# khiner/MeshEditor

Hardware: AMD Instinct MI355X
Metric: eigenpairs/sec (K/M assembly + 50-mode solve, 100k-tet mesh) (higher is better)
Workload: dtype f64; 1 GPU; cube_s100k: Kuhn mesh 105456 tets / 446631 DOF, NumModes=50 NumFemModes=65, P=10 excitation points, one mesh per GPU; eigenpairs_per_mesh=65, kept_modes_per_mesh=50, parallelism=mesh-per-gpu x1

## Files before the change

### mesheditor_amd/csrc/lab/mh_lab.hip

```cpp
#include "../mh_common.h"
#include "modalhip_lab.h"

#include <algorithm>

void mh_elementwise_apply(mh_context *ctx, const mh_system *sys, double sigma, const double *x, double *y, uint32_t w);

namespace {
constexpr int TB = 256;
__global__ void k_lab_ref_to_panel(const double *__restrict__ x, const uint32_t *__restrict__ perm, uint32_t nnodes, uint32_t width, double *__restrict__ panel) {
    const size_t i = size_t(blockIdx.x) * blockDim.x + threadIdx.x;
    if (i >= size_t(nnodes) * 3 * width) return;
    const uint32_t c = uint32_t(i % width), comp = uint32_t((i / width) % 3), node = uint32_t(i / (size_t(3) * width));
    panel[i] = x[size_t(c) * (size_t(3) * nnodes) + size_t(3) * perm[node] + comp];
}
__global__ void k_lab_panel_to_ref(const double *__restrict__ panel, const uint32_t *__restrict__ perm, uint32_t nnodes, uint32_t width, double *__restrict__ y) {
    const size_t i = size_t(blockIdx.x) * blockDim.x + threadIdx.x;
    if (i >= size_t(nnodes) * 3 * width) return;
    const uint32_t c = uint32_t(i % width), comp = uint32_t((i / width) % 3), node = uint32_t(i / (size_t(3) * width));
    y[size_t(c) * (size_t(3) * nnodes) + size_t(3) * perm[node] + comp] = panel[i];
}
}

namespace {
typedef float f4_stream __attribute__((ext_vector_type(4)));
// ... 223 lines not shown
    size_t bad = differing(one.x, hx);
    for (size_t r = 0; r < n; ++r)
        for (uint32_t c = 0; c < nc; ++c) {
            double ref = 0, mag = 0;
            for (uint32_t k = 0; k < m; ++k) {
                const double s = k < wa ? hx[r * b + map[k]] : k < wa + wb ? hw[r * wb + (k - wa)] : hp[r * wb + (k - wa - wb)];
                ref += s * hc[size_t(k) * nc + c];
                mag += std::abs(s * hc[size_t(k) * nc + c]);
            }
            const double got = c < wa ? one.xn[r * pitch + c] : one.p[r * wb + (c - wa)];
            bad += !(std::abs(got - ref) <= 2.0 * m * 2.3e-16 * mag);
        }
    std::vector<double> want = hx;
    size_t written = 0;
    for (size_t r = 0; r < n; ++r)
        for (uint32_t k = 0; k < wa; ++k) {
            want[r * b + map[k]] = one.xn[r * pitch + k];
            written += want[r * b + map[k]] != hx[r * b + map[k]];
        }
    if (written < n * wa / 2) mh_throw(MH_EHIP, "mapped update check: the update left %zu of %zu entries as they were", n * wa - written, n * size_t(wa));
    bad += differing(two.xn, one.xn) + differing(two.x, want) + differing(two.p, one.p);
    return double(bad);
}
}

extern "C" {
int mhl_context_bench_dense(mh_context *ctx, int kind, uint64_t n, uint32_t wa, uint32_t wb, uint32_t reps, double *avg_ms) {
    if (!ctx || !avg_ms || n == 0 || wa == 0 || wb == 0 || reps == 0 || kind < 0 || kind > 3) return MH_EINVAL;
    try {
        HIP_CHECK(hipSetDevice(ctx->device));
        std::lock_guard<std::mutex> lock(mh_solve_mutex());
        if (kind >= 2) {
            *avg_ms = lab_mapped_update_mismatches(ctx, kind == 3, n, wa, wb);
            return MH_OK;
        }
        DevArray<double> x(ctx, n * wa), y(ctx, n * wb), g(ctx, size_t(wa + wb) * (wa + wb)), z(ctx, n * wa);
        std::vector<double> h(n * std::max(wa, wb));
        for (size_t i = 0; i < h.size(); ++i) h[i] = double((i * 2654435761u) % 1000) * 1e-3 - 0.5;
        x.upload(h.data(), n * wa);
        y.upload(h.data(), n * wb);
        g.upload(h.data(), g.count);
        HIP_CHECK(hipStreamSynchronize(ctx->stream));
        auto run = [&]() {
            if (kind == 0) mh_gram(ctx, n, x, wa, y, wb, g, wa);
            else mh_combine(ctx, n, x, wa, y, wb, nullptr, 0, g, wa, z, wa, nullptr);
        };
        run();
        hipEvent_t e0, e1;
        HIP_CHECK(hipEventCreate(&e0));
        HIP_CHECK(hipEventCreate(&e1));
        HIP_CHECK(hipEventRecord(e0, ctx->stream));
        for (uint32_t r = 0; r < reps; ++r) run();
        HIP_CHECK(hipEventRecord(e1, ctx->stream));
// ... 513 lines not shown
```

### mesheditor_amd/csrc/mh_common.h

```cpp
#pragma once
#include "../../include/modalhip.h"

#include <hip/hip_runtime.h>
#include <rocblas/rocblas.h>
#include <rocsolver/rocsolver.h>

#include <algorithm>
#include <cstdarg>
#include <cstdio>
#include <cstdlib>
#include <cstring>
#include <iterator>
#include <limits>
#include <atomic>
#include <map>
#include <memory>
#include <mutex>
#include <stdexcept>
#include <string>
#include <vector>

struct MhError : std::runtime_error {
    int code;
    MhError(int c, const std::string &m) : std::runtime_error(m), code(c) {}
};

[[noreturn]] inline void mh_throw(int code, const char *fmt, ...) {
    char buf[512];
    va_list ap;
    va_start(ap, fmt);
    vsnprintf(buf, sizeof(buf), fmt, ap);
    va_end(ap);
    throw MhError(code, buf);
}

#define HIP_CHECK(expr)                                                                                         \
    do {                                                                                                        \
        hipError_t e_ = (expr);                                                                                 \
        if (e_ != hipSuccess) mh_throw(MH_EHIP, "%s failed: %s (%s:%d)", #expr, hipGetErrorString(e_), __FILE__, __LINE__); \
    } while (0)
#define ROCBLAS_CHECK(expr)                                                                                     \
    do {                                                                                                        \
// ... 175 lines not shown
        bytes_idle += it->second;
        live.erase(it);
        while (bytes_idle > cap && !free_blocks.empty()) {
            auto oldest = free_blocks.begin();
            for (auto f = free_blocks.begin(); f != free_blocks.end(); ++f)
                if (f->second.stamp < oldest->second.stamp) oldest = f;
            (void)hipFree(oldest->second.p);
            bytes_idle -= oldest->first;
            bytes_reserved -= oldest->first;
            free_blocks.erase(oldest);
        }
    }
    void trim() {
        for (auto &kv : free_blocks) (void)hipFree(kv.second.p), bytes_reserved -= kv.first;
        free_blocks.clear();
        bytes_idle = 0;
    }
    ~DevicePool() {
        trim();
        for (auto &kv : live) (void)hipFree(kv.first);
    }
};

struct mh_context {
    int device{0};
    int cu_count{256};
    hipStream_t stream{nullptr};
    hipStream_t aux_stream{nullptr};
    bool aux_stream_ready() {
        if (!aux_stream && hipStreamCreateWithFlags(&aux_stream, hipStreamNonBlocking) != hipSuccess) aux_stream = nullptr;
        if (aux_stream && !blas_aux) {
            if (rocblas_create_handle(&blas_aux) != rocblas_status_success) blas_aux = nullptr;
            else if (rocblas_set_stream(blas_aux, aux_stream) != rocblas_status_success) {
                (void)rocblas_destroy_handle(blas_aux);
                blas_aux = nullptr;
            }
        }
        return aux_stream != nullptr && blas_aux != nullptr;
    }
    hipStream_t aux2_stream{nullptr};
    std::vector<hipEvent_t> ahead_ev;
    bool aux2_stream_ready(size_t events = 0) {
        if (!aux2_stream && hipStreamCreateWithFlags(&aux2_stream, hipStreamNonBlocking) != hipSuccess) aux2_stream = nullptr, (void)hipGetLastError();
        while (aux2_stream && ahead_ev.size() < events) {
            hipEvent_t e = nullptr;
            if (hipEventCreateWithFlags(&e, hipEventDisableTiming) != hipSuccess) { (void)hipGetLastError(); return false; }
            ahead_ev.push_back(e);
        }
        return aux2_stream != nullptr;
    }
    rocblas_handle blas{nullptr};
    rocblas_handle blas_aux{nullptr};
    DevicePool pool;
    std::string last_error;
    hipEvent_t ev0{nullptr}, ev1{nullptr};
    void *gram_ws{nullptr};
    size_t gram_ws_bytes{0};
    uint32_t *iota{nullptr};
    unsigned long long *sytrd_xch{nullptr};
    uint32_t sytrd_epoch{0};
    int *sytrd_flag{nullptr};
    unsigned long long *sytrd_xch_wide{nullptr};
    uint32_t sytrd_epoch_wide{0};
    bool exchange_disabled{false};
    uint32_t sytrd_redos{0};
    unsigned long long *rr_check{nullptr};
    struct MhRrTrace *rr_trace{nullptr};
    bool time_kernels{false};
    std::vector<std::pair<hipEvent_t, hipEvent_t>> timer_events;
    std::vector<double> timer_work;
    std::vector<int> timer_class;
    size_t timer_used{0};
    struct ClassTotals {
        double ms{0}, work{0};
        uint64_t launches{0};
    } totals[MH_KERNEL_CLASSES];
// ... 5 lines not shown
    size_t slot{0};
    TimedLaunch(mh_context *c, int kernel_class, double work) : ctx(c), on(c->time_kernels) {
        if (!on) return;
        if (ctx->timer_used == ctx->timer_events.size()) {
            hipEvent_t a, b;
            HIP_CHECK(hipEventCreate(&a));
            HIP_CHECK(hipEventCreate(&b));
            ctx->timer_events.emplace_back(a, b);
            ctx->timer_work.push_back(0);
            ctx->timer_class.push_back(0);
        }
        slot = ctx->timer_used++;
        ctx->timer_work[slot] = work;
        ctx->timer_class[slot] = kernel_class;
        HIP_CHECK(hipEventRecord(ctx->timer_events[slot].first, ctx->stream));
    }
    ~TimedLaunch() {
        if (on) (void)hipEventRecord(ctx->timer_events[slot].second, ctx->stream);
    }
    TimedLaunch(const TimedLaunch &) = delete;
    TimedLaunch &operator=(const TimedLaunch &) = delete;
};

template<typename T> struct DevArray {
    mh_context *ctx{nullptr};
    T *ptr{nullptr};
    size_t count{0};
    bool owned{true};
    DevArray() = default;
    DevArray(mh_context *c, size_t n) { reset(c, n); }
    DevArray(const DevArray &) = delete;
    DevArray &operator=(const DevArray &) = delete;
    DevArray(DevArray &&o) noexcept : ctx(o.ctx), ptr(o.ptr), count(o.count), owned(o.owned) { o.ptr = nullptr; o.count = 0; o.owned = true; }
    DevArray &operator=(DevArray &&o) noexcept {
        if (this != &o) {
            free();
            ctx = o.ctx; ptr = o.ptr; count = o.count; owned = o.owned;
            o.ptr = nullptr; o.count = 0; o.owned = true;
        }
        return *this;
    }
    void alias_of(const DevArray &o) {
        free();
        ctx = o.ctx; ptr = o.ptr; count = o.count;
        owned = false;
    }
    ~DevArray() { free(); }
    void reset(mh_context *c, size_t n) {
        free();
        ctx = c;
        count = n;
        ptr = n ? static_cast<T *>(c->pool.alloc(n * sizeof(T))) : nullptr;
        static const bool poison = getenv("MH_TEST") && strstr(getenv("MH_TEST"), "poison");
        if (poison && ptr) (void)hipMemsetAsync(ptr, 0xff, n * sizeof(T), c->stream);
    }
    void free() {
        if (ptr && ctx && owned) ctx->pool.release(ptr);
        ptr = nullptr;
        count = 0;
        owned = true;
    }
    T *get() const { return ptr; }
    operator T *() const { return ptr; }
    void zero() const { if (ptr) HIP_CHECK(hipMemsetAsync(ptr, 0, count * sizeof(T), ctx->stream)); }
    void upload(const T *src, size_t n) const { HIP_CHECK(hipMemcpyAsync(ptr, src, n * sizeof(T), hipMemcpyHostToDevice, ctx->stream)); }
    void download(T *dst, size_t n) const {
        HIP_CHECK(hipMemcpyAsync(dst, ptr, n * sizeof(T), hipMemcpyDeviceToHost, ctx->stream));
        HIP_CHECK(hipStreamSynchronize(ctx->stream));
    }
    std::vector<T> to_host() const {
        std::vector<T> h(count);
        if (count) download(h.data(), count);
        return h;
    }
};

struct MhLevelStructure {
    uint32_t n_nodes{0};
    uint64_t n_blocks{0};
    DevArray<uint32_t> row_ptr, col;
    DevArray<uint32_t> seg, pay;
};
struct mh_structure {
    mh_context *ctx{nullptr};
    uint32_t n_points{0}, kept_tets{0}, n_nodes{0}, n_edges{0};
    DevArray<double> points;
    DevArray<uint32_t> tets;
    DevArray<uint32_t> elem_nodes_ref, elem_nodes, elem_p1;
    DevArray<double> elem_basis;
    DevArray<uint32_t> perm, inv_perm;
    bool relative{false};
    double origin[3]{0, 0, 0};
// ... 199 lines not shown
```

### mesheditor_amd/csrc/mh_dense.hip

```cpp
#include "mh_common.h"

#include <optional>

#include <map>

static bool mh_test_own_gemm() {
    static const bool on = getenv("MH_TEST") && strstr(getenv("MH_TEST"), "own_gemm");
    return on;
}
namespace {
constexpr int KC = 32;

typedef double double4_t __attribute__((ext_vector_type(4)));

__host__ __device__ inline int pad_pitch(int w) {
    int p = ((w + 15) / 16) * 16;
    if ((p % 32) != 16) p += 16;
    return p;
}

template<int TI, int TJ, int GI, int GJ, int KS, int OCC>
__global__ void __launch_bounds__(GI * GJ * KS * 64) __attribute__((amdgpu_waves_per_eu(OCC, OCC))) k_gram_blocked(const double *__restrict__ X, int ldx, int wa, const double *__restrict__ Y, int ldy, const uint32_t *__restrict__ ymap, int wb,
                                                                  size_t n, size_t rows_per_wg, double *__restrict__ partial) {
    extern __shared__ __attribute__((aligned(16))) double smem[];
// ... 1210 lines not shown
    if (multi && m >= 32) {
        constexpr int G = MH_SYTRD_GROUPS;
        constexpr size_t words = SYTRD_XCH_WORDS + SYTRD_ACK_WORDS;
        if (!ctx->sytrd_xch) {
            ctx->sytrd_xch = static_cast<unsigned long long *>(ctx->pool.alloc(words * sizeof(unsigned long long) + 64));
            HIP_CHECK(hipMemsetAsync(ctx->sytrd_xch, 0, words * sizeof(unsigned long long) + 64, ctx->stream));
        }
        if ((++ctx->sytrd_epoch & 0x7fffffu) == 0) {
            ctx->sytrd_epoch = 1;
            HIP_CHECK(hipMemsetAsync(ctx->sytrd_xch, 0, words * sizeof(unsigned long long) + 64, ctx->stream));
        }
        ctx->sytrd_flag = reinterpret_cast<int *>(ctx->sytrd_xch + words);
        HIP_CHECK(hipMemsetAsync(ctx->sytrd_flag, 0, sizeof(int), ctx->stream));
        k_sytrd_multi<G><<<8 * G, 256, 0, ctx->stream>>>(a, int(m), d, e, tau, ctx->sytrd_xch, ctx->sytrd_epoch, ctx->sytrd_flag);
    } else if (variant == 3) k_sytrd_regs<<<1, 512, 0, ctx->stream>>>(a, int(m), d, e, tau);
    else if (fused) k_sytrd_small_fused<<<1, MH_SYTRD_THREADS, 0, ctx->stream>>>(a, int(m), d, e, tau);
    else k_sytrd_small<<<1, 1024, 0, ctx->stream>>>(a, int(m), d, e, tau);
    KERNEL_CHECK();
}

bool mh_sytrd_gave_up(mh_context *ctx) {
    if (!ctx->sytrd_flag) return false;
    int flag = 0;
    HIP_CHECK(hipMemcpyAsync(&flag, ctx->sytrd_flag, sizeof(flag), hipMemcpyDeviceToHost, ctx->stream));
    HIP_CHECK(hipStreamSynchronize(ctx->stream));
    return flag != 0;
}

namespace {
template<int Q, int PF>
__global__ void __launch_bounds__(64) k_apply_q(const double *__restrict__ A, const double *__restrict__ tau, int m, double *__restrict__ Z, int ldz) {
    const int lane = threadIdx.x;
    double *zc = Z + size_t(blockIdx.x) * ldz;
    double z[Q], v[PF][Q], tk[PF];
#pragma unroll
    for (int q = 0; q < Q; ++q) z[q] = lane + 64 * q < m ? zc[lane + 64 * q] : 0.0;
    auto load = [&](int k, double (&dst)[Q], double &t) {
        t = k >= 0 ? tau[k] : 0.0;
#pragma unroll
        for (int q = 0; q < Q; ++q) {
            const int i = lane + 64 * q;
            dst[q] = (k >= 0 && i < m && i > k + 1) ? A[size_t(k) * m + i] : (i == k + 1 ? 1.0 : 0.0);
        }
    };
#pragma unroll
    for (int u = 0; u < PF; ++u) load(m - 2 - u, v[u], tk[u]);
    for (int k0 = m - 2; k0 >= 0; k0 -= PF) {
#pragma unroll
// ... 471 lines not shown
    if (m <= 256 || m > WIDE_T || k < 1 || k > 256 || k > m) return false;
    const size_t km = size_t(k) * m;
    double *xt = work, *xt2 = xt + km, *ufac = xt2 + km, *g = ufac + 3 * km, *linv = g + size_t(k) * k, *qual = linv + size_t(k) * k;
    k_tridiag_values<3><<<k, 256, 0, ctx->stream>>>(d, e, int(m), w);
    KERNEL_CHECK();
    k_tridiag_invit<<<div_up(k, 64), 64, 0, ctx->stream>>>(d, e, int(m), int(k), w, xt, ufac);
    KERNEL_CHECK();
    DevArray<int> info4_array(ctx, 4);
    int *info4 = info4_array.get();
    HIP_CHECK(hipMemsetAsync(info4, 0, 4 * sizeof(int), ctx->stream));
    for (int pass = 0; pass < 2; ++pass) {
        const double *src = pass == 0 ? xt : xt2;
        mh_small_gemm(ctx, false, true, k, k, m, 1.0, src, k, src, k, 0.0, g, k);
        mh_potrf(ctx, g, k, k, info4 + 2 * pass);
        HIP_CHECK(hipMemsetAsync(linv, 0, size_t(k) * k * sizeof(double), ctx->stream));
        ROCBLAS_CHECK(rocblas_dtrtri(ctx->blas, rocblas_fill_lower, rocblas_diagonal_non_unit, rocblas_int(k), g, rocblas_int(k), linv, rocblas_int(k)));
        if (pass == 0) mh_small_gemm(ctx, false, false, k, m, k, 1.0, linv, k, src, k, 0.0, xt2, k);
        else mh_small_gemm(ctx, true, true, m, k, k, 1.0, src, k, linv, k, 0.0, z, ldz);
    }
    HIP_CHECK(hipMemsetAsync(qual, 0, sizeof(double), ctx->stream));
    k_tridiag_residual<<<k, 256, 0, ctx->stream>>>(d, e, int(m), w, z, int(ldz), reinterpret_cast<unsigned long long *>(qual));
    KERNEL_CHECK();
    int hinfo[4] = {0, 0, 0, 0};
    HIP_CHECK(hipMemcpyAsync(quality_host, qual, sizeof(double), hipMemcpyDeviceToHost, ctx->stream));
    HIP_CHECK(hipMemcpyAsync(hinfo, info4, sizeof(hinfo), hipMemcpyDeviceToHost, ctx->stream));
    HIP_CHECK(hipStreamSynchronize(ctx->stream));
    if (hinfo[0] != 0 || hinfo[2] != 0) *quality_host = std::numeric_limits<double>::quiet_NaN();
    return true;
}

namespace {
__global__ void __launch_bounds__(256) k_potrf_small(double *__restrict__ A, int w, int *__restrict__ info) {
    extern __shared__ __attribute__((aligned(16))) double L[];
    __shared__ int s_fail;
    const int tid = threadIdx.x, pitch = w + 1;
    for (int idx = tid; idx < w * w; idx += 256) L[(idx / w) * pitch + idx % w] = A[idx];
    if (tid == 0) s_fail = 0;
    __syncthreads();
    for (int k = 0; k < w; ++k) {
        const double akk = L[k * pitch + k];
        if (!(akk > 0.0)) {
            if (tid == 0) s_fail = k + 1;
            break;
        }
        const double d = sqrt(akk), inv = 1.0 / d;
        __syncthreads();
        for (int i = k + tid; i < w; i += 256) L[k * pitch + i] = i == k ? d : L[k * pitch + i] * inv;
        __syncthreads();
        const int rem = w - k - 1;
// ... 382 lines not shown
```

### mesheditor_amd/csrc/mh_eigs.hip

```cpp
#include "mh_common.h"

#include <algorithm>
#include <cmath>
#include <memory>
#include <condition_variable>
#include <mutex>
#include <numeric>
#include <optional>
#include <type_traits>

__global__ void k_shift_values(const double *kval, const double *mval, size_t nblocks, double sigma, double *aval, float *aval32);
__global__ void k_diag_inverse(const uint32_t *row_ptr, const uint32_t *col, const double *aval, uint32_t nnodes, double *dinv);
__global__ void k_coarse_matrix(const uint32_t *row_ptr, const uint32_t *col, const double *aval, const double *tmat, const uint32_t *agg_of, const uint32_t *agg_ptr,
                                const uint32_t *agg_nodes, uint32_t nagg, double *a0);
__global__ void k_fix_coarse_diag(double *a0, uint32_t n0, double rel);

namespace {
constexpr int TB = 256;

std::mutex g_solve_mutex;
struct Switches {
    bool verbose = getenv("MH_VERBOSE") != nullptr;
    bool fp32_prec = !(getenv("MH_PRECOND_FP64") && atoi(getenv("MH_PRECOND_FP64")) != 0);
    int deg2 = 0, deg1 = 0, gamma = 0;
    double cheb_ratio = 0.0, cheb_ratio1 = 0.0;
    bool test_sytrd_giveup = getenv("MH_TEST") && strstr(getenv("MH_TEST"), "sytrd_giveup");
    bool no_tridiag_wide = getenv("MH_TEST") && strstr(getenv("MH_TEST"), "no_tridiag_wide");
    bool test_last_resort = getenv("MH_TEST") && strstr(getenv("MH_TEST"), "last_resort");
    bool test_coarse_pivot = getenv("MH_TEST") && strstr(getenv("MH_TEST"), "coarse_pivot");
    bool test_selfcheck_fail = getenv("MH_TEST") && strstr(getenv("MH_TEST"), "selfcheck_fail");
    bool lmax_low = getenv("MH_TEST") && strstr(getenv("MH_TEST"), "lmax_low");
    bool potrf_chain = getenv("MH_TEST") && strstr(getenv("MH_TEST"), "potrf_chain");
    bool no_poly_start = getenv("MH_TEST") && strstr(getenv("MH_TEST"), "no_poly_start");
    bool fresh_structure = getenv("MH_TEST") && strstr(getenv("MH_TEST"), "fresh_structure");
    bool copy_passes = getenv("MH_TEST") && strstr(getenv("MH_TEST"), "copy_passes");
    Switches() {
        if (const char *c = getenv("MH_CYCLE")) {
            double v[5] = {0, 0, 0, 0, 0};
            sscanf(c, "%lf,%lf,%lf,%lf,%lf", &v[0], &v[1], &v[2], &v[3], &v[4]);
            deg2 = std::max(0, int(v[0])), deg1 = std::max(0, int(v[1])), gamma = std::max(0, int(v[2]));
            cheb_ratio = v[3];
            cheb_ratio1 = v[4];
        }
    }
};
const Switches &switches() {
    static const Switches s;
    return s;
}
constexpr int kPowerIterations = 20;
constexpr uint32_t kPrecondColumns = 256;
constexpr uint32_t kSkipP = 4;
constexpr uint32_t kGuardPercent = 10;
constexpr float kFlatShape = 1e-4f;
constexpr size_t kDenseLastResort = 12288;
constexpr int kLastResortCg = 8;

struct PhaseLock {
// ... 572 lines not shown
bool sytrd_gave_up(mh_context *ctx, int flag, double *gA, const double *saved, uint32_t m) {
    if (!flag && !switches().test_sytrd_giveup) return false;
    ++ctx->sytrd_redos;
    HIP_CHECK(hipMemcpyAsync(gA, saved, size_t(m) * m * sizeof(double), hipMemcpyDeviceToDevice, ctx->stream));
    return true;
}
bool accept_partial(mh_context *ctx, double quality, double *evals, const double *lam, uint32_t nwant) {
    if (!(quality < 1e-10)) return false;
    HIP_CHECK(hipMemcpyAsync(evals, lam, size_t(nwant) * sizeof(double), hipMemcpyDeviceToDevice, ctx->stream));
    return true;
}

int eig_tridiag_small(mh_context *ctx, double *gA, uint32_t m, double *evals, double *ework, DevArray<int> &info, uint32_t nwant, std::vector<double> *host_evals) {
    DevArray<double> z(ctx, size_t(m) * m), tau(ctx, m);
    const bool partial = nwant && nwant < m;
    DevArray<double> zl(ctx, partial ? size_t(m) * nwant : 0);
    double *zres = z.get();
    uint32_t ncols = m;
    HIP_CHECK(hipMemcpyAsync(z.get(), gA, size_t(m) * m * sizeof(double), hipMemcpyDeviceToDevice, ctx->stream));
    for (int attempt = 0; attempt < 2; ++attempt) {
        mh_sytrd_small(ctx, gA, m, evals, ework, tau, attempt == 0 ? -1 : 0);
        int gave_up = 0;
        const bool flagged = attempt == 0 && ctx->sytrd_flag;
        if (flagged) HIP_CHECK(hipMemcpyAsync(&gave_up, ctx->sytrd_flag, sizeof(int), hipMemcpyDeviceToHost, ctx->stream));
        if (partial) {
            DevArray<double> wv(ctx, 2 * m + 8), ufac(ctx, size_t(3) * m * nwant);
            double *zout = attempt == 0 ? zl.get() : z.get();
            if (mh_tridiag_lowest(ctx, evals, ework, m, nwant, wv, zout, m, ufac, wv.get() + m, wv.get() + m + 8)) {
                double qv[5] = {1, 0, 0, 0, 0};
                std::vector<double> lam_host(host_evals ? nwant : 0);
                HIP_CHECK(hipMemcpyAsync(qv, wv.get() + m, sizeof(qv), hipMemcpyDeviceToHost, ctx->stream));
                if (host_evals) HIP_CHECK(hipMemcpyAsync(lam_host.data(), wv.get(), size_t(nwant) * sizeof(double), hipMemcpyDeviceToHost, ctx->stream));
                HIP_CHECK(hipStreamSynchronize(ctx->stream));
                if (flagged && sytrd_gave_up(ctx, gave_up, gA, z, m)) continue;
                if (switches().verbose)
                    fprintf(stderr, "[rr] tridiagonal m %u lowest %u: residual / ||T|| %.2e; us: multisection %.0f, inverse iteration %.0f, Gram-Schmidt %.0f, output %.0f\n", m,
                            nwant, qv[0], qv[1] * 0.01, qv[2] * 0.01, qv[3] * 0.01, qv[4] * 0.01);
                if (ctx->rr_trace) ctx->rr_trace->quality = qv[0];
                if (accept_partial(ctx, qv[0], evals, wv, nwant)) {
                    if (host_evals) host_evals->swap(lam_host);
                    zres = zout, ncols = nwant;
                    break;
                }
            }
        }
        if (flagged) {
            HIP_CHECK(hipStreamSynchronize(ctx->stream));
            if (sytrd_gave_up(ctx, gave_up, gA, z, m)) continue;
        }
        ROCBLAS_CHECK(rocsolver_dstedc(ctx->blas, rocblas_evect_tridiagonal, m, evals, ework, z, m, info));
        if (const int hinfo = host_info(info)) return hinfo;
        break;
    }
    if (ctx->rr_trace) ctx->rr_trace->solver = ncols < m ? MhRrTrace::SMALL_PARTIAL : MhRrTrace::SMALL_STEDC;
    mh_apply_q(ctx, gA, tau, m, zres, m, ncols);
    if (zres == zl.get()) rr_selfcheck(ctx, z.get(), m, zres, m, evals, ncols);
    HIP_CHECK(hipMemcpyAsync(gA, zres, size_t(m) * ncols * sizeof(double), hipMemcpyDeviceToDevice, ctx->stream));
    return 0;
}

std::optional<int> eig_tridiag_wide(mh_context *ctx, double *gA, uint32_t m, double *evals, double *ework, DevArray<int> &info, uint32_t nwant) {
    DevArray<double> z(ctx, size_t(m) * m), saved(ctx, size_t(m) * m), tau(ctx, m);
    HIP_CHECK(hipMemcpyAsync(saved.get(), gA, size_t(m) * m * sizeof(double), hipMemcpyDeviceToDevice, ctx->stream));
    mh_sytrd_wide(ctx, gA, m, evals, ework, tau);
    int gave_up = 0;
    HIP_CHECK(hipMemcpyAsync(&gave_up, ctx->sytrd_flag, sizeof(int), hipMemcpyDeviceToHost, ctx->stream));
    HIP_CHECK(hipStreamSynchronize(ctx->stream));
    if (sytrd_gave_up(ctx, gave_up, gA, saved, m)) return std::nullopt;
    if (nwant && nwant < m && nwant <= 256 && !switches().no_tridiag_wide) {
        DevArray<double> work(ctx, size_t(5) * nwant * m + size_t(2) * nwant * nwant + 8), lam(ctx, nwant);
        double quality = 1.0;
        if (mh_tridiag_lowest_wide(ctx, evals, ework, m, nwant, lam, z, m, work, info, &quality)) {
            if (switches().verbose) fprintf(stderr, "[rr] tridiagonal m %u lowest %u (wide): residual / ||T|| %.2e\n", m, nwant, quality);
            if (ctx->rr_trace) ctx->rr_trace->quality = quality;
            if (accept_partial(ctx, quality, evals, lam, nwant)) {
                if (ctx->rr_trace) ctx->rr_trace->solver = MhRrTrace::WIDE_PARTIAL;
                mh_apply_q(ctx, gA, tau, m, z, m, nwant);
                rr_selfcheck(ctx, saved.get(), m, z, m, evals, nwant);
                HIP_CHECK(hipMemcpyAsync(gA, z.get(), size_t(m) * nwant * sizeof(double), hipMemcpyDeviceToDevice, ctx->stream));
                HIP_CHECK(hipStreamSynchronize(ctx->stream));
                return 0;
            }
        }
    }
    ROCBLAS_CHECK(rocsolver_dstedc(ctx->blas, rocblas_evect_tridiagonal, m, evals, ework, z, m, info));
    if (const int hinfo = host_info(info)) return hinfo;
    ROCBLAS_CHECK(rocsolver_dormtr(ctx->blas, rocblas_side_left, rocblas_fill_lower, rocblas_operation_none, m, m, gA, m, tau, z, m));
    if (ctx->rr_trace) ctx->rr_trace->solver = MhRrTrace::WIDE_STEDC_ORMTR;
    HIP_CHECK(hipMemcpyAsync(gA, z.get(), size_t(m) * m * sizeof(double), hipMemcpyDeviceToDevice, ctx->stream));
    HIP_CHECK(hipStreamSynchronize(ctx->stream));
    return 0;
}

}

int mh_rr_solve(mh_context *ctx, double *gA, double *gM, uint32_t m, double *evals, double *ework, DevArray<int> &info, uint32_t nwant, bool gm_is_identity,
                std::vector<double> *host_evals) {
    const double one = 1, zero = 0;
    k_symmetrize_lower<<<grid1(size_t(m) * m), TB, 0, ctx->stream>>>(gA, m, m);
    KERNEL_CHECK();
    bool identity = gm_is_identity, series = false;
    if (!identity) {
        static_assert(sizeof(unsigned long long) == sizeof(double), "defect word");
        unsigned long long *defect = reinterpret_cast<unsigned long long *>(ework);
        HIP_CHECK(hipMemsetAsync(defect, 0, sizeof(unsigned long long), ctx->stream));
        k_identity_defect<<<grid1(size_t(m) * m), TB, 0, ctx->stream>>>(gM, m, defect);
        KERNEL_CHECK();
        unsigned long long bits = 0;
        HIP_CHECK(hipMemcpyAsync(&bits, defect, sizeof(bits), hipMemcpyDeviceToHost, ctx->stream));
        HIP_CHECK(hipStreamSynchronize(ctx->stream));
        double d;
        memcpy(&d, &bits, sizeof(d));
        identity = d < 1e-11;
        if (switches().verbose) fprintf(stderr, "[rr] m %u identity defect %.2e\n", m, d);
        series = !identity && d < 1e-7;
        if (ctx->rr_trace) ctx->rr_trace->defect = d;
    }
    if (ctx->rr_trace) ctx->rr_trace->reduction = gm_is_identity ? MhRrTrace::GIVEN_IDENTITY : identity ? MhRrTrace::MEASURED_IDENTITY : series ? MhRrTrace::SERIES : MhRrTrace::CHOLESKY;
    DevArray<double> sroot, stmp;
    if (series) {
        sroot.reset(ctx, size_t(m) * m);
        stmp.reset(ctx, size_t(m) * m * 2);
        double *e = stmp.get(), *e2 = stmp.get() + size_t(m) * m;
        k_defect_matrix<<<grid1(size_t(m) * m), TB, 0, ctx->stream>>>(gM, m, e);
        KERNEL_CHECK();
        small_dgemm(ctx, rocblas_operation_none, rocblas_operation_none, m, m, m, &one, e, m, e, m, &zero, e2, m);
        k_inverse_sqrt_series<<<grid1(size_t(m) * m), TB, 0, ctx->stream>>>(e, e2, m, sroot);
        KERNEL_CHECK();
        small_dgemm(ctx, rocblas_operation_none, rocblas_operation_none, m, m, m, &one, sroot, m, gA, m, &zero, e, m);
        small_dgemm(ctx, rocblas_operation_none, rocblas_operation_none, m, m, m, &one, e, m, sroot, m, &zero, gA, m);
        k_symmetrize_lower<<<grid1(size_t(m) * m), TB, 0, ctx->stream>>>(gA, m, m);
        KERNEL_CHECK();
        identity = true;
// ... 795 lines not shown
            std::swap(X, Xn); std::swap(AX, AXn); std::swap(MX, MXn);
            evals.download(theta.data(), b);
        }
    }

    bool converged_or_locked(uint32_t it) {
        if (cancel && *cancel) mh_throw(MH_ECANCELLED, "cancelled");
        if (g_concurrent) {
            iterating.release();
            iterating.acquire();
        }
        bool fused = res_ready;
        if (fused)
            for (const uint32_t i : res_act) fused = fused && !(std::abs(theta[i]) < 10.0 * std::abs(sigma));
        res_ready = false;
        rw_from_rr = fused;
        if (fused) {
            res_norms_d.download(res_norms.data(), size_t(2) * res_pitch);
            for (size_t k = 0; k < res_act.size(); ++k) {
                rn[res_act[k]] = res_norms[k];
                mn[res_act[k]] = res_norms[res_pitch + k];
            }
        } else {
        theta_d.upload(theta.data(), b);
        {
            const uint32_t rpb = 256, nblk = div_up(n, rpb);
            if (scratch.count < size_t(nblk) * 3 * b) scratch.reset(ctx, size_t(nblk) * 3 * b);
            dim3 grid(nblk, div_up(b, 64));
            k_residual_norms<<<grid, 64, 0, st>>>(AX, MX, X, theta_d, 10.0 * std::abs(sigma), R, n, b, rpb, scratch, scaled_norms ? sys->L2.dinv.get() : nullptr);
            KERNEL_CHECK();
            k_colsumsq_final<<<3 * b, 256, 0, st>>>(scratch, nblk, 3 * b, norms_d);
            KERNEL_CHECK();
            norms_d.download(norms.data(), 3 * size_t(b));
            std::copy(norms.begin(), norms.begin() + b, rn.begin());
            std::copy(norms.begin() + b, norms.begin() + 2 * b, mn.begin());
            std::copy(norms.begin() + 2 * b, norms.end(), xn.begin());
        }
        }
        act.clear();
        for (uint32_t i = 0; i < b; ++i) {
            const double rel = std::sqrt(rn[i]) / (std::abs(theta[i]) * std::sqrt(mn[i]));
            const bool near_shift = std::abs(theta[i]) < 10.0 * std::abs(sigma);
            const double floor_norm = scaled_norms ? sys->L2.lmax * std::sqrt(xn[i]) : anorm * std::sqrt(xn[i]);
            const double floor_factor = it == 0 && !warm && sys->worst_quality < kFlatShape ? 65536.0 : 256.0;
            const bool ok = rel < residual_tol || (near_shift && std::sqrt(rn[i]) < floor_factor * 2.2e-16 * floor_norm);
            if (ok) locked[i] = 1;
            if (!locked[i]) act.push_back(i);
// ... 31 lines not shown
                if (!locked[i]) worst_active = std::max(worst_active, std::sqrt(rn[i]) / (std::abs(theta[i]) * std::sqrt(mn[i])));
            }
            best_worst_active = std::min(best_worst_active, worst_active);
            hist_active.push_back(worst_active);
            if (inner_cg > 0 && it >= 40) {
                const size_t h = hist_active.size();
                if (h > 30 && hist_nconv[h - 31] == nconv && worst_active > 0.9 * hist_active[h - 31] && worst_active <= 10.0 * residual_tol) {
                    pairs_at_floor = nev > nconv ? nev - nconv : 0;
                    if (verbose) fprintf(stderr, "[lobpcg] it %3u: %u pairs have sat at a residual of %.2e (tolerance %.1e) for thirty iterations -- the rounding floor of this mesh; handed on as they are\n", it, pairs_at_floor, worst_active, residual_tol);
                    converged = true;
                    return true;
                }
            }
            floor_strikes = it >= 20 && worst_active > 1e3 * best_worst_active ? floor_strikes + 1 : 0;
            if (floor_strikes >= 3)
                mh_throw(MH_ENOTCONVERGED, "LOBPCG: %u of %u pairs converged; the others sit at the rounding floor (residual %.1e and growing, best %.1e, tolerance %.1e)", nconv, nev,
                         worst_active, best_worst_active, residual_tol);
        }
        return false;
    }

    void search_directions(uint32_t it) {
        w = uint32_t(act.size());
        idx_d.upload(act.data(), w);
        const double *residuals = Rw.get();
        const bool in_place = precondition_reads_columns(w);
        uint32_t r_pitch = 0;
        const uint32_t *r_map = nullptr;
        if (rw_from_rr) {
            if (act == res_act && res_pitch == w) {
                residuals = Rr.get();
            } else {
                std::vector<uint32_t> &pos = res_pos;
                pos.assign(w, 0);
                size_t q = 0;
                for (uint32_t k = 0; k < w; ++k) {
                    while (q < res_act.size() && res_act[q] != act[k]) ++q;
                    if (q == res_act.size()) mh_throw(MH_EHIP, "active column %u was not active before", act[k]);
                    pos[k] = uint32_t(q);
                }
                pos_d.upload(pos.data(), w);
                if (in_place) {
                    residuals = Rr.get(), r_pitch = res_pitch, r_map = pos_d;
                } else {
                    k_gather_cols<<<grid1(n * w), TB, 0, st>>>(Rr, pos_d, Rw, n, res_pitch, w);
                    KERNEL_CHECK();
                }
            }
        } else if (in_place) {
            residuals = R.get(), r_pitch = b, r_map = idx_d;
        } else {
            k_gather_cols<<<grid1(n * w), TB, 0, st>>>(R, idx_d, Rw, n, b, w);
            KERNEL_CHECK();
        }
        for (uint32_t k = 0; k < w; ++k) theta_act[k] = theta[act[k]];
        theta_act_d.upload(theta_act.data(), w);
        {
            Timer tp(ctx);
            precondition(residuals, W, w, r_pitch, r_map);
            precond_seconds += tp.stop();
            prof.op_applications += w;
        }
        bool ok = true;
        p_implicit = false;
        if (pproj_ok && wp) {
            gram(ctx, n, MX, b, W, w, H, b);
            mh_pack_stacked(ctx, H, b, nullptr, 0, w, -1.0, Ct);
            mh_combine(ctx, n, X, b, nullptr, 0, nullptr, 0, Ct, w, W, w, nullptr, true);
            mh_spmm(ctx, sys->L2, sys->L2.aval, W, AW, sys->L2.mval, MW, w);
            gram(ctx, n, P, wp, MW, w, Hp, wp);
            lazy_images = true;
            w_implicit = false;
            ok = chol_orthonormalise(W, MW, AW, w, false, true, Hp, wp);
            if (!ok) mh_throw(MH_ENOTCONVERGED, "search directions lost rank at iteration %u", it);
            if (p_needs_explicit) {
                mh_pack_stacked(ctx, Hp, wp, nullptr, 0, w, -1.0, Ct);
                mh_combine(ctx, n, P, wp, nullptr, 0, nullptr, 0, Ct, w, W, w, nullptr, true);
                mh_spmm(ctx, sys->L2, sys->L2.aval, W, AW, sys->L2.mval, MW, w);
                lazy_images = w <= 256;
// ... 161 lines not shown
                dim3 grid(nblk, div_up(w2, 64));
                k_colsum_partial<<<grid, 64, 0, st>>>(res_partial, sys->n_nodes, w2, res_blocks, rpb);
                KERNEL_CHECK();
                k_colsumsq_final<<<w2, 256, 0, st>>>(res_blocks, nblk, w2, res_norms_d);
                KERNEL_CHECK();
                res_act = act;
                res_pitch = pitch;
                res_ready = true;
            } else {
                mh_spmm_mapped(ctx, sys->L2, sys->L2.aval, Xn, AX, sys->L2.mval, MX, pitch, b, wa, idx_d);
            }
        }
        std::swap(P, Pn); std::swap(MP, MPn);
        wp = wp_new;
    }

    void finish(double *eigenvalues) {
        prof.restarts = iters;
        prof.op_solve = precond_seconds;
        if (!converged) mh_throw(MH_ENOTCONVERGED, "LOBPCG: %u of %u pairs converged in %u iterations", nconv, nev, iters);
        for (uint32_t k = 0; k < nev; ++k) eigenvalues[k] = theta[order[k]] + sigma;
        sys->plain_residual = -1.0;
        if (scaled_norms) {
            theta_d.upload(theta.data(), b);
            const uint32_t rpb = 256, nblk = div_up(n, rpb);
            if (scratch.count < size_t(nblk) * 3 * b) scratch.reset(ctx, size_t(nblk) * 3 * b);
            k_residual_norms<<<dim3(nblk, div_up(b, 64)), 64, 0, st>>>(AX, MX, X, theta_d, 10.0 * std::abs(sigma), R, n, b, rpb, scratch, nullptr);
            KERNEL_CHECK();
            k_colsumsq_final<<<3 * b, 256, 0, st>>>(scratch, nblk, 3 * b, norms_d);
            KERNEL_CHECK();
            norms_d.download(norms.data(), 3 * size_t(b));
            double worst = 0;
            for (uint32_t k = 0; k < nev; ++k) {
                const uint32_t i = order[k];
                if (std::abs(theta[i]) < 10.0 * std::abs(sigma)) continue;
                worst = std::max(worst, std::sqrt(norms[i]) / (std::abs(theta[i]) * std::sqrt(norms[b + i])));
            }
            sys->plain_residual = worst;
            if (verbose) fprintf(stderr, "[lobpcg] accepted in the Jacobi-scaled norm at %.1e; worst elastic pair in the plain 2-norm: %.2e\n", residual_tol, worst);
        }
        sys->evecs.reset(ctx, n * nev);
        sys->evec_cols = nev;
        idx_d.upload(order.data(), nev);
        k_gather_cols<<<grid1(n * nev), TB, 0, st>>>(X, idx_d, sys->evecs, n, b, nev);
        KERNEL_CHECK();
        HIP_CHECK(hipStreamSynchronize(st));
        prof.iterate = t_iter.stop();
        read_health();
        sys->profile = prof;
        if (profile) *profile = prof;
        if (switches().test_selfcheck_fail && !ctx->exchange_disabled) prof.rr_selfcheck = 1.0;
        if (!(prof.rr_selfcheck < 1e-6))
            mh_throw(MH_EHIP, "Rayleigh-Ritz self-check failed: a step's eigenpairs leave a relative residual of %.2e against the step's own matrix", prof.rr_selfcheck);
    }
    void read_health() {
        prof.sytrd_redos = ctx->sytrd_redos - redos_at_start;
        prof.pairs_at_floor = pairs_at_floor;
        prof.rr_selfcheck = 0.0;
        if (ctx->rr_check) {
            unsigned long long bits = 0;
            HIP_CHECK(hipMemcpyAsync(&bits, ctx->rr_check, sizeof(bits), hipMemcpyDeviceToHost, st));
            HIP_CHECK(hipStreamSynchronize(st));
            memcpy(&prof.rr_selfcheck, &bits, sizeof(double));
        }
    }

    void run(double *eigenvalues) {
        start();
        for (uint32_t it = 0; it <= max_iters; ++it) {
            if (converged_or_locked(it)) break;
            search_directions(it);
            rayleigh_ritz(it);
            conjugate_directions(it);
            update_basis(it);
        }
        finish(eigenvalues);
    }
};
struct Attempt {
    mh_system *sys;
    uint32_t nev, b;
    double sigma, residual_tol;
    const float *seed;
    uint32_t srows, scols;
    const volatile unsigned char *cancel;
// ... 228 lines not shown
```

Baseline: 645.6 eigenpairs/s.

## Replace small device-host copies with a pinned mailbox ring and host spin-wait

Adds a mapped pinned-memory mailbox ring. Small read-backs become a tiny copy kernel that writes into host-visible memory and bumps a sequence word, and the host spin-waits on that word instead of issuing hipMemcpyAsync plus hipStreamSynchronize. Small uploads are staged through the same mapped slots by a copy kernel, and the LOBPCG search step now batches its index, theta and position uploads into one staged transfer. The aim is to cut per-transfer runtime latency on the many small synchronising transfers in the iterative solver. In exchange it burns a host core while spinning, depends on fence and visibility semantics of mapped memory, and falls back to a stream sync when a deadline passes.

```diff
diff --git a/mesheditor_amd/csrc/lab/mh_lab.hip b/mesheditor_amd/csrc/lab/mh_lab.hip
--- a/mesheditor_amd/csrc/lab/mh_lab.hip
+++ b/mesheditor_amd/csrc/lab/mh_lab.hip
@@ -269,13 +269,50 @@
     bad += differing(two.xn, one.xn) + differing(two.x, want) + differing(two.p, one.p);
     return double(bad);
 }
+__global__ void k_lab_fill_from_ticket(uint32_t *out, uint32_t words, uint32_t cycle) {
+    for (uint32_t i = threadIdx.x; i < words; i += blockDim.x) out[i] = cycle * 2654435761u + i;
+}
+__global__ void k_lab_wait_ms(double ms, unsigned long long *sink) {
+    const long long t0 = wall_clock64(), ticks = (long long)(ms * 1e5);
+    unsigned long long spins = 0;
+    while (wall_clock64() - t0 < ticks && spins < (1ull << 24)) {
+        ++spins;
+        __builtin_amdgcn_s_sleep(32);
+    }
+    if (spins == ~0ull) *sink = spins;
+}
+double lab_mailbox_mismatches(mh_context *ctx, size_t cycles, uint32_t words, uint32_t every) {
+    if (size_t(words) * 4 > MhMailboxRing::kSlotBytes) mh_throw(MH_EINVAL, "a payload of %u words exceeds a mailbox slot", words);
+    DevArray<uint32_t> payload(ctx, words);
+    DevArray<unsigned long long> sink(ctx, 1);
+    std::vector<uint32_t> got(words);
+    size_t bad = 0;
+    for (size_t c = 1; c <= cycles; ++c) {
+        if (every && c % every == 0) {
+            k_lab_wait_ms<<<1, 1, 0, ctx->stream>>>(2.0, sink);
+            KERNEL_CHECK();
+        }
+        k_lab_fill_from_ticket<<<1, 256, 0, ctx->stream>>>(payload, words, uint32_t(c));
+        KERNEL_CHECK();
+        std::fill(got.begin(), got.end(), 0u);
+        mh_read_back(ctx, {{got.data(), payload.get(), size_t(words) * 4}});
+        for (uint32_t i = 0; i < words; ++i) bad += got[i] != uint32_t(c) * 2654435761u + i;
+    }
+    if (!mh_blit_readbacks() && ctx->mailbox.waits < cycles) mh_throw(MH_EHIP, "mailbox check: %zu cycles but %llu waits", cycles, (unsigned long long)ctx->mailbox.waits);
+    HIP_CHECK(hipStreamSynchronize(ctx->stream));
+    return double(bad);
+}
 }
 
 extern "C" {
 int mhl_context_bench_dense(mh_context *ctx, int kind, uint64_t n, uint32_t wa, uint32_t wb, uint32_t reps, double *avg_ms) {
-    if (!ctx || !avg_ms || n == 0 || wa == 0 || wb == 0 || reps == 0 || kind < 0 || kind > 3) return MH_EINVAL;
-    try {
-        HIP_CHECK(hipSetDevice(ctx->device));
+    if (!ctx || !avg_ms || n == 0 || wa == 0 || wb == 0 || reps == 0 || kind < 0 || kind > 4) return MH_EINVAL;
+    try {
+        HIP_CHECK(hipSetDevice(ctx->device));
+        if (kind == 4) {
+            *avg_ms = lab_mailbox_mismatches(ctx, n, wa, wb <= n ? wb : 0);
+            return MH_OK;
+        }
         std::lock_guard<std::mutex> lock(mh_solve_mutex());
         if (kind >= 2) {
             *avg_ms = lab_mapped_update_mismatches(ctx, kind == 3, n, wa, wb);
diff --git a/mesheditor_amd/csrc/mh_common.h b/mesheditor_amd/csrc/mh_common.h
--- a/mesheditor_amd/csrc/mh_common.h
+++ b/mesheditor_amd/csrc/mh_common.h
@@ -1,5 +1,6 @@
 #pragma once
 #include "../../include/modalhip.h"
+#include "mh_mailbox.h"
 
 #include <hip/hip_runtime.h>
 #include <rocblas/rocblas.h>
@@ -18,6 +19,7 @@
 #include <mutex>
 #include <stdexcept>
 #include <string>
+#include <initializer_list>
 #include <vector>
 
 struct MhError : std::runtime_error {
@@ -239,6 +241,39 @@
     }
 };
 
+inline bool mh_test_has(const char *word) { return getenv("MH_TEST") && strstr(getenv("MH_TEST"), word); }
+inline bool mh_blit_readbacks() {
+    static const bool on = mh_test_has("blit_readbacks");
+    return on;
+}
+constexpr std::chrono::nanoseconds kMailboxDeadline = std::chrono::milliseconds(53);
+struct MhMailbox {
+    MhMailboxRing ring;
+    char *host{nullptr}, *host_seen_by_device{nullptr};
+    uint64_t waits{0}, staged{0}, deadline_ends{0}, no_token_ends{0}, longest_wait_ns{0};
+    static constexpr size_t kBytes = MhMailboxRing::kSlots * (MhMailboxRing::kSlotBytes + 64);
+    void ensure() {
+        if (host) return;
+        HIP_CHECK(hipHostMalloc(reinterpret_cast<void **>(&host), kBytes, hipHostMallocMapped));
+        memset(host, 0, kBytes);
+        HIP_CHECK(hipHostGetDevicePointer(reinterpret_cast<void **>(&host_seen_by_device), host, 0));
+    }
+    char *slot(uint32_t s) const { return host + size_t(s) * MhMailboxRing::kSlotBytes; }
+    char *slot_seen_by_device(uint32_t s) const { return host_seen_by_device + size_t(s) * MhMailboxRing::kSlotBytes; }
+    static constexpr size_t seq_offset(uint32_t s) { return MhMailboxRing::kSlots * MhMailboxRing::kSlotBytes + size_t(s) * 64; }
+    volatile uint32_t *seq_word(uint32_t s) const { return reinterpret_cast<volatile uint32_t *>(host + seq_offset(s)); }
+    volatile uint32_t *seq_word_seen_by_device(uint32_t s) const { return reinterpret_cast<volatile uint32_t *>(host_seen_by_device + seq_offset(s)); }
+    MhMailbox() = default;
+    MhMailbox(const MhMailbox &) = delete;
+    MhMailbox &operator=(const MhMailbox &) = delete;
+    ~MhMailbox() {
+        if (host && mh_test_has("mailbox_stats"))
+            fprintf(stderr, "[mailbox] %llu read-backs (longest wait %.1f us; %llu ended at the deadline, %llu without the spin token), %llu staged uploads\n",
+                    (unsigned long long)waits, longest_wait_ns * 1e-3, (unsigned long long)deadline_ends, (unsigned long long)no_token_ends, (unsigned long long)staged);
+        if (host) (void)hipHostFree(host);
+    }
+};
+
 struct mh_context {
     int device{0};
     int cu_count{256};
@@ -269,6 +304,7 @@
     rocblas_handle blas{nullptr};
     rocblas_handle blas_aux{nullptr};
     DevicePool pool;
+    MhMailbox mailbox;
     std::string last_error;
     hipEvent_t ev0{nullptr}, ev1{nullptr};
     void *gram_ws{nullptr};
@@ -320,6 +356,100 @@
     TimedLaunch &operator=(const TimedLaunch &) = delete;
 };
 
+struct MhWordCopy {
+    const uint32_t *src[4];
+    uint32_t *dst[4];
+    uint32_t words[4];
+};
+#if defined(__HIPCC__)
+template<int BLOCK> __global__ void __launch_bounds__(BLOCK) k_mailbox_copy(MhWordCopy c, volatile uint32_t *seq_word, uint32_t seq) {
+    for (int p = 0; p < 4; ++p)
+        for (uint32_t i = threadIdx.x; i < c.words[p]; i += BLOCK) c.dst[p][i] = c.src[p][i];
+    if (!seq_word) return;
+    __threadfence_system();
+    __syncthreads();
+    if (threadIdx.x == 0) {
+        *seq_word = seq;
+        __threadfence_system();
+    }
+}
+#endif
+struct MhTransfer {
+    void *dst;
+    const void *src;
+    size_t bytes;
+};
+inline bool mh_mailbox_takes(std::initializer_list<MhTransfer> parts) {
+    size_t total = 0;
+    for (const MhTransfer &p : parts) {
+        if (p.bytes % 4 || reinterpret_cast<uintptr_t>(p.src) % 4 || reinterpret_cast<uintptr_t>(p.dst) % 4) return false;
+        total += (p.bytes + 7) & ~size_t(7);
+    }
+    return parts.size() <= 4 && total <= MhMailboxRing::kSlotBytes;
+}
+inline void mh_read_back(mh_context *ctx, std::initializer_list<MhTransfer> parts) {
+#if defined(__HIPCC__)
+    if (!mh_blit_readbacks() && mh_mailbox_takes(parts)) {
+        MhMailbox &mb = ctx->mailbox;
+        mb.ensure();
+        const uint64_t ticket = mb.ring.take();
+        const uint32_t s = MhMailboxRing::slot_of(ticket);
+        MhWordCopy c{};
+        size_t off = 0, k = 0;
+        for (const MhTransfer &p : parts) {
+            c.src[k] = static_cast<const uint32_t *>(p.src);
+            c.dst[k] = reinterpret_cast<uint32_t *>(mb.slot_seen_by_device(s) + off);
+            c.words[k++] = uint32_t(p.bytes / 4);
+            off += (p.bytes + 7) & ~size_t(7);
+        }
+        k_mailbox_copy<256><<<1, 256, 0, ctx->stream>>>(c, mb.seq_word_seen_by_device(s), uint32_t(ticket));
+        KERNEL_CHECK();
+        static const bool one_spinner = !mh_test_has("mailbox_every_thread_spins");
+        uint64_t waited = 0;
+        const MhWaitEnd end = mh_mailbox_wait(mb.seq_word(s), uint32_t(ticket), kMailboxDeadline, one_spinner, [&] { HIP_CHECK(hipStreamSynchronize(ctx->stream)); }, &waited);
+        mb.ring.saw(ticket);
+        ++mb.waits;
+        mb.deadline_ends += end == MhWaitEnd::DEADLINE, mb.no_token_ends += end == MhWaitEnd::NO_TOKEN;
+        mb.longest_wait_ns = std::max(mb.longest_wait_ns, waited);
+        off = 0;
+        for (const MhTransfer &p : parts) {
+            if (p.bytes) memcpy(p.dst, mb.slot(s) + off, p.bytes);
+            off += (p.bytes + 7) & ~size_t(7);
+        }
+        return;
+    }
+#endif
+    for (const MhTransfer &p : parts)
+        if (p.bytes) HIP_CHECK(hipMemcpyAsync(p.dst, p.src, p.bytes, hipMemcpyDeviceToHost, ctx->stream));
+    HIP_CHECK(hipStreamSynchronize(ctx->stream));
+}
+inline void mh_stage_in(mh_context *ctx, std::initializer_list<MhTransfer> parts) {
+#if defined(__HIPCC__)
+    if (!mh_blit_readbacks() && mh_mailbox_takes(parts)) {
+        MhMailbox &mb = ctx->mailbox;
+        mb.ensure();
+        const uint64_t ticket = mb.ring.take();
+        const uint32_t s = MhMailboxRing::slot_of(ticket);
+        MhWordCopy c{};
+        size_t off = 0, k = 0;
+        for (const MhTransfer &p : parts) {
+            if (p.bytes) memcpy(mb.slot(s) + off, p.src, p.bytes);
+            c.src[k] = reinterpret_cast<const uint32_t *>(mb.slot_seen_by_device(s) + off);
+            c.dst[k] = static_cast<uint32_t *>(p.dst);
+            c.words[k++] = uint32_t(p.bytes / 4);
+            off += (p.bytes + 7) & ~size_t(7);
+        }
+        std::atomic_thread_fence(std::memory_order_release);
+        k_mailbox_copy<256><<<1, 256, 0, ctx->stream>>>(c, nullptr, 0);
+        KERNEL_CHECK();
+        ++mb.staged;
+        return;
+    }
+#endif
+    for (const MhTransfer &p : parts)
+        if (p.bytes) HIP_CHECK(hipMemcpyAsync(p.dst, p.src, p.bytes, hipMemcpyHostToDevice, ctx->stream));
+}
+
 template<typename T> struct DevArray {
     mh_context *ctx{nullptr};
     T *ptr{nullptr};
@@ -362,10 +492,7 @@
     operator T *() const { return ptr; }
     void zero() const { if (ptr) HIP_CHECK(hipMemsetAsync(ptr, 0, count * sizeof(T), ctx->stream)); }
     void upload(const T *src, size_t n) const { HIP_CHECK(hipMemcpyAsync(ptr, src, n * sizeof(T), hipMemcpyHostToDevice, ctx->stream)); }
-    void download(T *dst, size_t n) const {
-        HIP_CHECK(hipMemcpyAsync(dst, ptr, n * sizeof(T), hipMemcpyDeviceToHost, ctx->stream));
-        HIP_CHECK(hipStreamSynchronize(ctx->stream));
-    }
+    void download(T *dst, size_t n) const { mh_read_back(ctx, {{dst, ptr, n * sizeof(T)}}); }
     std::vector<T> to_host() const {
         std::vector<T> h(count);
         if (count) download(h.data(), count);
diff --git a/mesheditor_amd/csrc/mh_dense.hip b/mesheditor_amd/csrc/mh_dense.hip
--- a/mesheditor_amd/csrc/mh_dense.hip
+++ b/mesheditor_amd/csrc/mh_dense.hip
@@ -1256,8 +1256,7 @@
 bool mh_sytrd_gave_up(mh_context *ctx) {
     if (!ctx->sytrd_flag) return false;
     int flag = 0;
-    HIP_CHECK(hipMemcpyAsync(&flag, ctx->sytrd_flag, sizeof(flag), hipMemcpyDeviceToHost, ctx->stream));
-    HIP_CHECK(hipStreamSynchronize(ctx->stream));
+    mh_read_back(ctx, {{&flag, ctx->sytrd_flag, sizeof(flag)}});
     return flag != 0;
 }
 
@@ -1775,9 +1774,7 @@
     k_tridiag_residual<<<k, 256, 0, ctx->stream>>>(d, e, int(m), w, z, int(ldz), reinterpret_cast<unsigned long long *>(qual));
     KERNEL_CHECK();
     int hinfo[4] = {0, 0, 0, 0};
-    HIP_CHECK(hipMemcpyAsync(quality_host, qual, sizeof(double), hipMemcpyDeviceToHost, ctx->stream));
-    HIP_CHECK(hipMemcpyAsync(hinfo, info4, sizeof(hinfo), hipMemcpyDeviceToHost, ctx->stream));
-    HIP_CHECK(hipStreamSynchronize(ctx->stream));
+    mh_read_back(ctx, {{quality_host, qual, sizeof(double)}, {hinfo, info4, sizeof(hinfo)}});
     if (hinfo[0] != 0 || hinfo[2] != 0) *quality_host = std::numeric_limits<double>::quiet_NaN();
     return true;
 }
diff --git a/mesheditor_amd/csrc/mh_eigs.hip b/mesheditor_amd/csrc/mh_eigs.hip
--- a/mesheditor_amd/csrc/mh_eigs.hip
+++ b/mesheditor_amd/csrc/mh_eigs.hip
@@ -34,6 +34,7 @@
     bool no_poly_start = getenv("MH_TEST") && strstr(getenv("MH_TEST"), "no_poly_start");
     bool fresh_structure = getenv("MH_TEST") && strstr(getenv("MH_TEST"), "fresh_structure");
     bool copy_passes = getenv("MH_TEST") && strstr(getenv("MH_TEST"), "copy_passes");
+    bool blit_readbacks = mh_blit_readbacks();
     Switches() {
         if (const char *c = getenv("MH_CYCLE")) {
             double v[5] = {0, 0, 0, 0, 0};
@@ -652,16 +653,17 @@
         mh_sytrd_small(ctx, gA, m, evals, ework, tau, attempt == 0 ? -1 : 0);
         int gave_up = 0;
         const bool flagged = attempt == 0 && ctx->sytrd_flag;
-        if (flagged) HIP_CHECK(hipMemcpyAsync(&gave_up, ctx->sytrd_flag, sizeof(int), hipMemcpyDeviceToHost, ctx->stream));
+        bool flag_read = false;
         if (partial) {
             DevArray<double> wv(ctx, 2 * m + 8), ufac(ctx, size_t(3) * m * nwant);
             double *zout = attempt == 0 ? zl.get() : z.get();
             if (mh_tridiag_lowest(ctx, evals, ework, m, nwant, wv, zout, m, ufac, wv.get() + m, wv.get() + m + 8)) {
                 double qv[5] = {1, 0, 0, 0, 0};
                 std::vector<double> lam_host(host_evals ? nwant : 0);
-                HIP_CHECK(hipMemcpyAsync(qv, wv.get() + m, sizeof(qv), hipMemcpyDeviceToHost, ctx->stream));
-                if (host_evals) HIP_CHECK(hipMemcpyAsync(lam_host.data(), wv.get(), size_t(nwant) * sizeof(double), hipMemcpyDeviceToHost, ctx->stream));
-                HIP_CHECK(hipStreamSynchronize(ctx->stream));
+                mh_read_back(ctx, {{qv, wv.get() + m, sizeof(qv)},
+                                   {lam_host.data(), wv.get(), host_evals ? size_t(nwant) * sizeof(double) : 0},
+                                   {&gave_up, ctx->sytrd_flag, flagged ? sizeof(int) : 0}});
+                flag_read = flagged;
                 if (flagged && sytrd_gave_up(ctx, gave_up, gA, z, m)) continue;
                 if (switches().verbose)
                     fprintf(stderr, "[rr] tridiagonal m %u lowest %u: residual / ||T|| %.2e; us: multisection %.0f, inverse iteration %.0f, Gram-Schmidt %.0f, output %.0f\n", m,
@@ -675,7 +677,7 @@
             }
         }
         if (flagged) {
-            HIP_CHECK(hipStreamSynchronize(ctx->stream));
+            if (!flag_read) mh_read_back(ctx, {{&gave_up, ctx->sytrd_flag, sizeof(int)}});
             if (sytrd_gave_up(ctx, gave_up, gA, z, m)) continue;
         }
         ROCBLAS_CHECK(rocsolver_dstedc(ctx->blas, rocblas_evect_tridiagonal, m, evals, ework, z, m, info));
@@ -694,8 +696,7 @@
     HIP_CHECK(hipMemcpyAsync(saved.get(), gA, size_t(m) * m * sizeof(double), hipMemcpyDeviceToDevice, ctx->stream));
     mh_sytrd_wide(ctx, gA, m, evals, ework, tau);
     int gave_up = 0;
-    HIP_CHECK(hipMemcpyAsync(&gave_up, ctx->sytrd_flag, sizeof(int), hipMemcpyDeviceToHost, ctx->stream));
-    HIP_CHECK(hipStreamSynchronize(ctx->stream));
+    mh_read_back(ctx, {{&gave_up, ctx->sytrd_flag, sizeof(int)}});
     if (sytrd_gave_up(ctx, gave_up, gA, saved, m)) return std::nullopt;
     if (nwant && nwant < m && nwant <= 256 && !switches().no_tridiag_wide) {
         DevArray<double> work(ctx, size_t(5) * nwant * m + size_t(2) * nwant * nwant + 8), lam(ctx, nwant);
@@ -737,8 +738,7 @@
         k_identity_defect<<<grid1(size_t(m) * m), TB, 0, ctx->stream>>>(gM, m, defect);
         KERNEL_CHECK();
         unsigned long long bits = 0;
-        HIP_CHECK(hipMemcpyAsync(&bits, defect, sizeof(bits), hipMemcpyDeviceToHost, ctx->stream));
-        HIP_CHECK(hipStreamSynchronize(ctx->stream));
+        mh_read_back(ctx, {{&bits, defect, sizeof(bits)}});
         double d;
         memcpy(&d, &bits, sizeof(d));
         identity = d < 1e-11;
@@ -1580,7 +1580,7 @@
                 mn[res_act[k]] = res_norms[res_pitch + k];
             }
         } else {
-        theta_d.upload(theta.data(), b);
+        mh_stage_in(ctx, {{theta_d.get(), theta.data(), b * sizeof(double)}});
         {
             const uint32_t rpb = 256, nblk = div_up(n, rpb);
             if (scratch.count < size_t(nblk) * 3 * b) scratch.reset(ctx, size_t(nblk) * 3 * b);
@@ -1658,30 +1658,33 @@
 
     void search_directions(uint32_t it) {
         w = uint32_t(act.size());
-        idx_d.upload(act.data(), w);
+        for (uint32_t k = 0; k < w; ++k) theta_act[k] = theta[act[k]];
+        const bool with_pos = rw_from_rr && !(act == res_act && res_pitch == w);
+        if (with_pos) {
+            std::vector<uint32_t> &pos = res_pos;
+            pos.assign(w, 0);
+            size_t q = 0;
+            for (uint32_t k = 0; k < w; ++k) {
+                while (q < res_act.size() && res_act[q] != act[k]) ++q;
+                if (q == res_act.size()) mh_throw(MH_EHIP, "active column %u was not active before", act[k]);
+                pos[k] = uint32_t(q);
+            }
+        }
+        mh_stage_in(ctx, {{idx_d.get(), act.data(), w * sizeof(uint32_t)},
+                          {theta_act_d.get(), theta_act.data(), w * sizeof(double)},
+                          {pos_d.get(), res_pos.data(), with_pos ? w * sizeof(uint32_t) : 0}});
         const double *residuals = Rw.get();
         const bool in_place = precondition_reads_columns(w);
         uint32_t r_pitch = 0;
         const uint32_t *r_map = nullptr;
         if (rw_from_rr) {
-            if (act == res_act && res_pitch == w) {
+            if (!with_pos) {
                 residuals = Rr.get();
+            } else if (in_place) {
+                residuals = Rr.get(), r_pitch = res_pitch, r_map = pos_d;
             } else {
-                std::vector<uint32_t> &pos = res_pos;
-                pos.assign(w, 0);
-                size_t q = 0;
-                for (uint32_t k = 0; k < w; ++k) {
-                    while (q < res_act.size() && res_act[q] != act[k]) ++q;
-                    if (q == res_act.size()) mh_throw(MH_EHIP, "active column %u was not active before", act[k]);
-                    pos[k] = uint32_t(q);
-                }
-                pos_d.upload(pos.data(), w);
-                if (in_place) {
-                    residuals = Rr.get(), r_pitch = res_pitch, r_map = pos_d;
-                } else {
-                    k_gather_cols<<<grid1(n * w), TB, 0, st>>>(Rr, pos_d, Rw, n, res_pitch, w);
-                    KERNEL_CHECK();
-                }
+                k_gather_cols<<<grid1(n * w), TB, 0, st>>>(Rr, pos_d, Rw, n, res_pitch, w);
+                KERNEL_CHECK();
             }
         } else if (in_place) {
             residuals = R.get(), r_pitch = b, r_map = idx_d;
@@ -1689,8 +1692,6 @@
             k_gather_cols<<<grid1(n * w), TB, 0, st>>>(R, idx_d, Rw, n, b, w);
             KERNEL_CHECK();
         }
-        for (uint32_t k = 0; k < w; ++k) theta_act[k] = theta[act[k]];
-        theta_act_d.upload(theta_act.data(), w);
         {
             Timer tp(ctx);
             precondition(residuals, W, w, r_pitch, r_map);
@@ -1898,7 +1899,7 @@
         for (uint32_t k = 0; k < nev; ++k) eigenvalues[k] = theta[order[k]] + sigma;
         sys->plain_residual = -1.0;
         if (scaled_norms) {
-            theta_d.upload(theta.data(), b);
+            mh_stage_in(ctx, {{theta_d.get(), theta.data(), b * sizeof(double)}});
             const uint32_t rpb = 256, nblk = div_up(n, rpb);
             if (scratch.count < size_t(nblk) * 3 * b) scratch.reset(ctx, size_t(nblk) * 3 * b);
             k_residual_norms<<<dim3(nblk, div_up(b, 64)), 64, 0, st>>>(AX, MX, X, theta_d, 10.0 * std::abs(sigma), R, n, b, rpb, scratch, nullptr);
@@ -1917,7 +1918,7 @@
         }
         sys->evecs.reset(ctx, n * nev);
         sys->evec_cols = nev;
-        idx_d.upload(order.data(), nev);
+        mh_stage_in(ctx, {{idx_d.get(), order.data(), nev * sizeof(uint32_t)}});
         k_gather_cols<<<grid1(n * nev), TB, 0, st>>>(X, idx_d, sys->evecs, n, b, nev);
         KERNEL_CHECK();
         HIP_CHECK(hipStreamSynchronize(st));
@@ -1935,8 +1936,7 @@
         prof.rr_selfcheck = 0.0;
         if (ctx->rr_check) {
             unsigned long long bits = 0;
-            HIP_CHECK(hipMemcpyAsync(&bits, ctx->rr_check, sizeof(bits), hipMemcpyDeviceToHost, st));
-            HIP_CHECK(hipStreamSynchronize(st));
+            mh_read_back(ctx, {{&bits, ctx->rr_check, sizeof(bits)}});
             memcpy(&prof.rr_selfcheck, &bits, sizeof(double));
         }
     }
diff --git a/mesheditor_amd/csrc/mh_mailbox.h b/mesheditor_amd/csrc/mh_mailbox.h
--- /dev/null
+++ b/mesheditor_amd/csrc/mh_mailbox.h
@@ -0,0 +1,71 @@
+#pragma once
+#include <atomic>
+#include <chrono>
+#include <cstddef>
+#include <cstdint>
+#include <stdexcept>
+
+struct MhMailboxRing {
+    static constexpr uint32_t kSlots = 16;
+    static constexpr size_t kSlotBytes = 4096;
+    uint64_t issued{0}, observed{0};
+    uint64_t take() {
+        const uint64_t t = issued + 1;
+        if (t > kSlots && observed <= t - kSlots) throw std::logic_error("read-back mailbox: a slot would be rewritten before a later ticket was observed");
+        return issued = t;
+    }
+    void saw(uint64_t t) {
+        if (t > observed) observed = t;
+    }
+    static uint32_t slot_of(uint64_t t) { return uint32_t(t % kSlots); }
+};
+
+struct MhSpinToken {
+    static std::atomic<bool> &taken() {
+        static std::atomic<bool> t{false};
+        return t;
+    }
+    bool held;
+    explicit MhSpinToken(bool exclusive) : held(!exclusive || !taken().exchange(true, std::memory_order_acquire)), owns(exclusive && held) {}
+    ~MhSpinToken() {
+        if (owns) taken().store(false, std::memory_order_release);
+    }
+    MhSpinToken(const MhSpinToken &) = delete;
+    MhSpinToken &operator=(const MhSpinToken &) = delete;
+
+  private:
+    bool owns;
+};
+
+enum class MhWaitEnd { SEEN = 0, DEADLINE = 1, NO_TOKEN = 2 };
+template<typename Fallback>
+MhWaitEnd mh_mailbox_wait(const volatile uint32_t *seq_word, uint32_t want, std::chrono::nanoseconds deadline, bool one_spinner, Fallback &&fallback,
+                          uint64_t *waited_ns = nullptr) {
+    MhWaitEnd end = MhWaitEnd::SEEN;
+    if (waited_ns) *waited_ns = 0;
+    if (*seq_word != want) {
+        MhSpinToken token(one_spinner);
+        if (!token.held) {
+            fallback();
+            end = MhWaitEnd::NO_TOKEN;
+        } else {
+            const auto t0 = std::chrono::steady_clock::now();
+            for (;;) {
+                bool seen = false;
+                for (int i = 0; i < 64 && !(seen = *seq_word == want); ++i) __builtin_ia32_pause();
+                const auto dt = std::chrono::steady_clock::now() - t0;
+                if (seen) {
+                    if (waited_ns) *waited_ns = uint64_t(std::chrono::duration_cast<std::chrono::nanoseconds>(dt).count());
+                    break;
+                }
+                if (dt > deadline) {
+                    fallback();
+                    end = MhWaitEnd::DEADLINE;
+                    break;
+                }
+            }
+        }
+    }
+    std::atomic_thread_fence(std::memory_order_acquire);
+    return end;
+}
```

Result: no change. 649.8 eigenpairs/s, median of 6 (+0.7%).
